# crispitagorico/sigkernel

Hardware: AMD Instinct MI355X
Metric: Gram entries/sec (fp64) (higher is better)
Workload: dtype f64; 1 GPU; BASELINE configs[2]: batch 512x512, len 128, dim 8, LinearKernel, dyadic 1, fp64, compute_Gram sym=False; step=compute_Gram, batch_x=512, rows_per_gpu=512, batch_y=512, len_x=128, len_y=128, dim=8, static_kernel=linear, dyadic_order=1, parallelism=SigKernel(process_group): gram rows sharded over 1 GPU(s), 1 all-gather per Gram

## Files before the change

### include/sigkernel_amd.h

```cpp
#ifndef SIGKERNEL_AMD_H
#define SIGKERNEL_AMD_H

#include <stddef.h>
#include <stdint.h>

#ifdef __cplusplus
extern "C" {
#endif

typedef enum sk_status {
    SK_OK = 0,
    SK_ERR_BAD_ARG = 1,
    SK_ERR_UNSUPPORTED = 2,
    SK_ERR_LAUNCH = 3,
    SK_ERR_WORKSPACE = 4,
    SK_ERR_NO_DEVICE = 5
} sk_status;

#define SK_SCHEME_DEFAULT 0
#define SK_SCHEME_NAIVE 1

#define SK_FLAG_NONE 0
#define SK_FLAG_EXACT 1
#define SK_FLAG_SIMPLE 2
#define SK_FLAG_EDGES_GIVEN 8
#define SK_FLAG_FAST_ONLY 4

int sk_version(void);
const char *sk_build_info(void);

#define SK_ROUTE_NO_STREAM 1
#define SK_ROUTE_NO_SWAP 2
double sk_cost_query(int which);
const char *sk_cost_name(int which);
const char *sk_cost_note(int which);
#define SK_OP_FORWARD 0
#define SK_OP_ADJOINT 1
#define SK_OP_ADJOINT_SYM 2
#define SK_OP_PREFIX 3
#define SK_OP_TRUNCATED 4
#define SK_OP_TRUNCATED_ADJOINT 5
#define SK_OP_TRUNCATED_RBF 6
#define SK_OP_TRUNCATED_RBF_ADJOINT 7
#define SK_OP_TRUNCATED_LONG 8
#define SK_OP_TRUNCATED_LONG_ADJOINT 9
#define SK_OP_TRUNCATED_WIDE_ADJOINT 10
#define SK_ROUTE_STREAM 0
#define SK_ROUTE_FUSED 1
#define SK_ROUTE_FUSED_MB 2
#define SK_ROUTE_FUSED_MB_SWAP 3
#define SK_ROUTE_FUSED_SWAP 4
int sk_route_query(int op, int kind, int D, int M, int N, int dyadic, int scheme, int elem_size, int flags);

void sk_reload_knobs(void);

int sk_launch_trace(int enable);
size_t sk_launch_trace_dump(char *buf, size_t n, int reset);

double sk_linear_prescale(int dyadic);
const char *sk_status_string(int status);
int sk_device_count(void);

int sk_increments_f64(const double *G, int64_t P, int M, int N, double *inc_c, int64_t ld, void *stream);
int sk_increments_f32(const float *G, int64_t P, int M, int N, float *inc_c, int64_t ld, void *stream);

int sk_static_increments_f64(int kind, double param, const double *X, const double *Y, int64_t A, int64_t B, int M, int N,
                             int D, double *inc_c, int64_t ld, void *stream);
int sk_static_increments_f32(int kind, double param, const float *X, const float *Y, int64_t A, int64_t B, int M, int N,
                             int D, float *inc_c, int64_t ld, void *stream);

int sk_static_adjoint_f64(int kind, double param, const double *X, const double *Y, const double *W, int64_t ldw,
                          const double *scale, int64_t A, int64_t B, int M, int N, int D, double *out, void *stream);
int sk_static_adjoint_f32(int kind, double param, const float *X, const float *Y, const float *W, int64_t ldw,
                          const float *scale, int64_t A, int64_t B, int M, int N, int D, float *out, void *stream);

int sk_linear_adjoint_f64(const double *dYt, int64_t ldy, const double *W, int64_t ldw, const double *scale, int64_t A,
                          int64_t B, int Mc, int Nc, int D, double *out, void *stream);
int sk_linear_adjoint_f32(const double *dYt, int64_t ldy, const float *W, int64_t ldw, const float *scale, int64_t A, int64_t B,
                          int Mc, int Nc, int D, float *out, void *stream);

int sk_linear_adjoint_fused_f64(const double *dXr, const double *dYt, int64_t A, int64_t B, int Mrows, int Mc, int Nc, int Ncp,
                                int dyadic, int scheme, const double *edges, const double *scale, double *tpart,
                                size_t tpart_doubles, double *err, double *ypart, size_t ypart_doubles, int *ppg_out, int *rows_out,
                                int *ycols_out, const double *kfinal, double screen, double tol, void *rescue_ws,
                                size_t rescue_ws_bytes, void *stream);

int sk_rbf_adjoint_fused_f64(const double *Xr, const double *Yt, int64_t A, int64_t B, int Mrows, int Mc, int Nc, int Ncp, int D,
                             int dyadic, int scheme, double sigma, const double *edges, const double *scale, double *gpart,
                             size_t gpart_doubles, double *err, double *ypart, size_t ypart_doubles, int *ppg_out, int *rows_out,
                             int *outw_out, int *ycols_out, const double *kfinal, double screen, double tol, void *rescue_ws,
                             size_t rescue_ws_bytes, void *stream);

size_t sk_solve_deriv_static_workspace_bytes(int64_t P, int Mc, int Nc, int dyadic, int D, int *mrows);
int sk_solve_deriv_static_f64(int kind, double param, const double *X0r, const double *X1r, const double *X2r, const double *Yt, int64_t A,
                              int64_t B, int Mrows, int Mc, int Nc, int Ncp, int D, int fd, int dyadic, int scheme, double eps, double *out_k,
                              double *out_kd, double *out_kdd, void *workspace, size_t workspace_bytes, void *stream);

int sk_rbf_adjoint_fused_mb_layout(int64_t P, int Mc, int Nc, int dyadic, int D, int *mrows, int *rows, int *outw, int *ncols,
                                   int64_t *edge_doubles, size_t *workspace_bytes);
int sk_rbf_adjoint_fused_mb_f64(const double *Xr, const void *Yt, int yt_f32, int64_t A, int64_t B, int Mrows, int Mc, int Nc, int Ncp, int D, int fd,
                                int dyadic, int scheme, double sigma, const double *edges, const double *scale, double *gpart,
                                size_t gpart_doubles, double *n0, size_t n0_doubles, double *err, void *workspace, size_t workspace_bytes,
                                const double *yt64, const double *kfinal, double screen, double tol, void *rescue_ws, size_t rescue_ws_bytes,
                                void *stream);

int sk_linear_adjoint_fused_mb_layout(int64_t P, int Mc, int Nc, int dyadic, int D, int *mrows, int *rows, int *outw, int64_t *edge_doubles,
                                      size_t *workspace_bytes);
int sk_linear_adjoint_fused_mb_f64(const double *dXr, const double *dYt, int64_t A, int64_t B, int Mrows, int Mc, int Nc, int Ncp, int D, int fd,
                                   int dyadic, int scheme, const double *edges, const double *scale, double *gpart, size_t gpart_doubles,
                                   double *err, void *workspace, size_t workspace_bytes, const double *kfinal, double screen, double tol,
                                   void *rescue_ws, size_t rescue_ws_bytes, void *stream);

// ... 199 lines not shown
```

### sigkernel_amd/_lib.py

```python
import ctypes
import os

import torch

from ._routes import routes

_HERE = os.path.dirname(os.path.abspath(__file__))
LIB_PATH = os.path.join(_HERE, "libsigkernel_amd.so")

SK_OK = 0
OP_FORWARD, OP_ADJOINT, OP_ADJOINT_SYM, OP_PREFIX, OP_TRUNCATED, OP_TRUNCATED_ADJOINT, OP_TRUNCATED_RBF = 0, 1, 2, 3, 4, 5, 6
OP_TRUNCATED_RBF_ADJOINT = 7
OP_TRUNCATED_LONG = 8
OP_TRUNCATED_LONG_ADJOINT = 9
OP_TRUNCATED_WIDE_ADJOINT = 10
ROUTE_STREAM, ROUTE_FUSED, ROUTE_FUSED_MB, ROUTE_FUSED_MB_SWAP, ROUTE_FUSED_SWAP = 0, 1, 2, 3, 4
ROUTE_NO_STREAM = 1
ROUTE_NO_SWAP = 2
SCHEME_DEFAULT = 0
SCHEME_NAIVE = 1
FLAG_EXACT = 1
FLAG_SIMPLE = 2
FLAG_FAST_ONLY = 4
FLAG_EDGES_GIVEN = 8
PREFIX_NODES = {"all": 0, "diagonal": 1, "last_row": 2, "last_col": 3}


def prefix_nodes_len(nodes, M, N):
    return {"diagonal": min(M, N), "last_row": N, "last_col": M}[nodes]

_lib = None

_vp = ctypes.c_void_p
_i64 = ctypes.c_int64
_int = ctypes.c_int
_sz = ctypes.c_size_t

SIGNATURES = {
    "sk_version": (_int, []),
    "sk_build_info": (ctypes.c_char_p, []),
    "sk_route_query": (_int, [_int, _int, _int, _int, _int, _int, _int, _int, _int]),
    "sk_cost_query": (ctypes.c_double, [_int]),
    "sk_cost_name": (ctypes.c_char_p, [_int]),
    "sk_cost_note": (ctypes.c_char_p, [_int]),
    "sk_solve_fwd_static_cols": (_int, [_int, _int]),
    "sk_reload_knobs": (None, []),
    "sk_launch_trace": (_int, [_int]),
    "sk_launch_trace_dump": (ctypes.c_size_t, [ctypes.c_char_p, ctypes.c_size_t, _int]),
    "sk_linear_prescale": (ctypes.c_double, [_int]),
    "sk_status_string": (ctypes.c_char_p, [_int]),
    "sk_device_count": (_int, []),
    "sk_increments_f64": (_int, [_vp, _i64, _int, _int, _vp, _i64, _vp]),
    "sk_increments_f32": (_int, [_vp, _i64, _int, _int, _vp, _i64, _vp]),
    "sk_static_increments_f64": (_int, [_int, ctypes.c_double, _vp, _vp, _i64, _i64, _int, _int, _int, _vp, _i64, _vp]),
    "sk_static_increments_f32": (_int, [_int, ctypes.c_double, _vp, _vp, _i64, _i64, _int, _int, _int, _vp, _i64, _vp]),
    "sk_static_adjoint_f64": (_int, [_int, ctypes.c_double, _vp, _vp, _vp, _i64, _vp, _i64, _i64, _int, _int, _int, _vp, _vp]),
    "sk_static_adjoint_f32": (_int, [_int, ctypes.c_double, _vp, _vp, _vp, _i64, _vp, _i64, _i64, _int, _int, _int, _vp, _vp]),
    "sk_linear_adjoint_f64": (_int, [_vp, _i64, _vp, _i64, _vp, _i64, _i64, _int, _int, _int, _vp, _vp]),
    "sk_linear_adjoint_f32": (_int, [_vp, _i64, _vp, _i64, _vp, _i64, _i64, _int, _int, _int, _vp, _vp]),
    "sk_static_adjoint2_f64": (_int, [_int, ctypes.c_double, _vp, _vp, _vp, _int, _vp, _i64, _vp, _i64, _i64, _int, _int, _int, _int,
                                      _vp, _vp]),
    "sk_static_adjoint2_f32": (_int, [_int, ctypes.c_double, _vp, _vp, _vp, _int, _vp, _i64, _vp, _i64, _i64, _int, _int, _int, _int,
                                      _vp, _vp]),
    "sk_increments_adjoint_f64": (_int, [_vp, _i64, _vp, _i64, _int, _int, _vp, _vp]),
    "sk_increments_adjoint_f32": (_int, [_vp, _i64, _vp, _i64, _int, _int, _vp, _vp]),
    "sk_solve_fwd_f64": (_int, [_vp, _i64, _i64, _int, _int, _int, _int, _int, _vp, _vp, _vp, _vp]),
    "sk_solve_fwd_f32": (_int, [_vp, _i64, _i64, _int, _int, _int, _int, _int, _vp, _vp, _vp, _vp]),
    "sk_solve_fwd_linear_f64": (_int, [_vp, _vp, _i64, _i64, _int, _int, _int, _int, _int, _int, _int, _vp, _vp, _vp]),
    "sk_solve_fwd_linear_f32": (_int, [_vp, _vp, _i64, _i64, _int, _int, _int, _int, _int, _int, _int, _vp, _vp, _vp]),
    "sk_solve_fwd_rbf_f64": (_int, [_vp, _vp, _i64, _i64, _int, _int, _int, _int, _int, _int, _int, ctypes.c_double, _vp, _vp, _vp]),
    "sk_solve_fwd_rbf_f32": (_int, [_vp, _vp, _i64, _i64, _int, _int, _int, _int, _int, _int, _int, ctypes.c_double, _vp, _vp, _vp]),
    "sk_solve_prefix_linear_f64": (_int, [_vp, _vp, _i64, _i64, _int, _int, _int, _int, _int, _int, _int, _vp, _i64, _vp, _vp]),
    "sk_solve_prefix_linear_f32": (_int, [_vp, _vp, _i64, _i64, _int, _int, _int, _int, _int, _int, _int, _vp, _i64, _vp, _vp]),
    "sk_solve_prefix_rbf_f64": (_int, [_vp, _vp, _i64, _i64, _int, _int, _int, _int, _int, _int, _int, ctypes.c_double, _vp, _i64, _vp, _vp]),
    "sk_solve_prefix_rbf_f32": (_int, [_vp, _vp, _i64, _i64, _int, _int, _int, _int, _int, _int, _int, ctypes.c_double, _vp, _i64, _vp, _vp]),
    "sk_solve_prefix_nodes_linear_f64": (_int, [_vp, _vp, _i64, _i64, _int, _int, _int, _int, _int, _int, _int, _int, _vp, _i64, _vp, _vp]),
    "sk_solve_prefix_nodes_linear_f32": (_int, [_vp, _vp, _i64, _i64, _int, _int, _int, _int, _int, _int, _int, _int, _vp, _i64, _vp, _vp]),
    "sk_solve_prefix_nodes_rbf_f64": (_int, [_vp, _vp, _i64, _i64, _int, _int, _int, _int, _int, _int, _int, ctypes.c_double, _int, _vp, _i64, _vp, _vp]),
    "sk_solve_prefix_nodes_rbf_f32": (_int, [_vp, _vp, _i64, _i64, _int, _int, _int, _int, _int, _int, _int, ctypes.c_double, _int, _vp, _i64, _vp, _vp]),
    "sk_solve_prefix_at_linear_f64": (_int, [_vp, _vp, _i64, _i64, _int, _int, _int, _int, _int, _int, _int, _vp, _vp, _vp, _vp, _vp]),
    "sk_solve_prefix_at_linear_f32": (_int, [_vp, _vp, _i64, _i64, _int, _int, _int, _int, _int, _int, _int, _vp, _vp, _vp, _vp, _vp]),
    "sk_solve_prefix_at_rbf_f64": (_int, [_vp, _vp, _i64, _i64, _int, _int, _int, _int, _int, _int, _int, ctypes.c_double, _vp, _vp, _vp, _vp, _vp]),
    "sk_solve_prefix_at_rbf_f32": (_int, [_vp, _vp, _i64, _i64, _int, _int, _int, _int, _int, _int, _int, ctypes.c_double, _vp, _vp, _vp, _vp, _vp]),
    "sk_truncated_gram_f64": (_int, [_vp, _vp, _i64, _i64, _int, _int, _int, _int, _int, _int, _int, _int, _vp, _vp, _vp]),
    "sk_truncated_gram_f32": (_int, [_vp, _vp, _i64, _i64, _int, _int, _int, _int, _int, _int, _int, _int, _vp, _vp, _vp]),
    "sk_truncated_paired_f64": (_int, [_vp, _vp, _i64, _int, _int, _int, _int, _int, _int, _int, _int, _vp, _vp, _vp]),
    "sk_truncated_paired_f32": (_int, [_vp, _vp, _i64, _int, _int, _int, _int, _int, _int, _int, _int, _vp, _vp, _vp]),
    "sk_truncated_levels_f64": (_int, [_vp, _vp, _i64, _i64, _int, _int, _int, _int, _int, _int, _int, _int, _vp, _vp]),
    "sk_truncated_levels_f32": (_int, [_vp, _vp, _i64, _i64, _int, _int, _int, _int, _int, _int, _int, _int, _vp, _vp]),
    "sk_truncated_levels_paired_f64": (_int, [_vp, _vp, _i64, _int, _int, _int, _int, _int, _int, _int, _int, _vp, _vp]),
    "sk_truncated_levels_paired_f32": (_int, [_vp, _vp, _i64, _int, _int, _int, _int, _int, _int, _int, _int, _vp, _vp]),
    "sk_truncated_points_f64": (_int, [_vp, _vp, _i64, _i64, _int, _int, _int, _int, _int, _int, _int, _int, _int, ctypes.c_double, _int, _int, _vp, _vp, _vp]),
    "sk_truncated_points_f32": (_int, [_vp, _vp, _i64, _i64, _int, _int, _int, _int, _int, _int, _int, _int, _int, ctypes.c_double, _int, _int, _vp, _vp, _vp]),
    "sk_truncated_long_plan": (_int, [_i64, _i64, _int, _int, _int, _int, _int, _sz, _vp]),
    "sk_truncated_long_f64": (_int, [_vp, _vp, _i64, _i64, _int, _int, _int, _int, _int, _int, _int, _int, _int, _int, _vp, _vp, _sz, _vp, _vp]),
    "sk_truncated_long_f32": (_int, [_vp, _vp, _i64, _i64, _int, _int, _int, _int, _int, _int, _int, _int, _int, _int, _vp, _vp, _sz, _vp, _vp]),
    "sk_truncated_adjoint_plan": (_int, [_i64, _i64, _int, _int, _int, _int, _int, _sz, _vp]),
    "sk_truncated_long_adjoint_plan": (_int, [_i64, _i64, _int, _int, _int, _int, _int, _sz, _vp]),
    "sk_truncated_long_adjoint": (_int, [_vp, _vp, _i64, _i64, _int, _int, _int, _int, _int, _int, _int, _vp, _vp, _i64, _vp, _sz, _vp, _int]),
    "sk_truncated_wide_adjoint_plan": (_int, [_i64, _i64, _int, _int, _int, _int, _int, _sz, _vp]),
    "sk_truncated_wide_adjoint": (_int, [_vp, _vp, _i64, _i64, _int, _int, _int, _int, _int, _int, _int, _vp, _vp, _i64, _vp, _sz, _vp, _int]),
    "sk_truncated_adjoint": (_int, [_vp, _vp, _i64, _i64, _int, _int, _int, _int, _int, _int, _int, _vp, _vp, _i64, _vp, _sz, _vp, _int]),
# ... 1447 lines not shown
```

### sigkernel_amd/csrc/sk_pair_stream.h

```cpp
#pragma once
#include "sk_wave_common.h"

namespace sk {
namespace {

__device__ __forceinline__ void lds_read_dims_issue(d2_t (&t)[8], unsigned a_even, unsigned a_odd) {
    asm volatile("ds_read_b128 %0, %8\n\t"
                 "ds_read_b128 %1, %9\n\t"
                 "ds_read_b128 %2, %8 offset:256\n\t"
                 "ds_read_b128 %3, %9 offset:256\n\t"
                 "ds_read_b128 %4, %8 offset:512\n\t"
                 "ds_read_b128 %5, %9 offset:512\n\t"
                 "ds_read_b128 %6, %8 offset:768\n\t"
                 "ds_read_b128 %7, %9 offset:768"
                 : "=&v"(t[0]), "=&v"(t[1]), "=&v"(t[2]), "=&v"(t[3]), "=&v"(t[4]), "=&v"(t[5]), "=&v"(t[6]), "=&v"(t[7])
                 : "v"(a_even), "v"(a_odd)
                 : "memory");
}
__device__ __forceinline__ void lds_read_dims_issue(d2_t (&t)[4], unsigned a_even, unsigned a_odd) {
    asm volatile("ds_read_b128 %0, %4\n\t"
                 "ds_read_b128 %1, %5\n\t"
                 "ds_read_b128 %2, %4 offset:256\n\t"
                 "ds_read_b128 %3, %5 offset:256"
                 : "=&v"(t[0]), "=&v"(t[1]), "=&v"(t[2]), "=&v"(t[3])
// ... 39 lines not shown
template <bool TRI, int FD, class PRM>
__device__ __forceinline__ int64_t pair_split(const PRM &prm, int64_t p, bool want_b) {
    if (prm.B <= 0) return p;
    if constexpr (TRI) {
        if (prm.tri) {
            const int *tab = reinterpret_cast<const int *>(prm.dYt + prm.B * (int64_t)FD * prm.Ncp);
            return (int64_t)tab[2 * p + (want_b ? 1 : 0)];
        }
    }
    if (want_b) return (int64_t)((uint32_t)p % (uint32_t)prm.B);
    return (int64_t)((uint32_t)p / (uint32_t)prm.B);
}


constexpr int x_window(int kind, int nd, int rc, bool edges) { return (kind == 0 && nd == 8 && rc == 4 && !edges) ? 4 : 8; }
constexpr int y_slab_pitch(int nd) { return nd * 128; }
constexpr int X_SLOTS = 2;
constexpr int x_row_bytes(int nd) { return nd == 4 ? 32 : 64; }

struct OneBandGeom {
    int NUp, logL, L, G, JMAX, GY;
    bool shy;
    size_t lds_bytes;
    int64_t n_pos;
};
struct OneBandShape {
    int kind, Mc, Nc, Mrows, Ncp, RC, nd;
    bool edges;
    int64_t A, B, P;
    int tri, logL_fixed;
};
inline int one_band_geometry(const OneBandShape &in, OneBandGeom &o) {
    const int NU = in.kind == 1 ? (in.Nc + 2) / 2 : (in.Nc + 1) / 2;
    const int rows = in.kind == 1 ? in.Mc + 1 : in.Mc;
    o.NUp = (NU + LINE_UNITS - 1) / LINE_UNITS * LINE_UNITS;
    if (in.Ncp < o.NUp * 2 || (in.Ncp & 1)) return SK_ERR_UNSUPPORTED;
    o.logL = 3;
    while (o.logL < 6 && (in.RC << o.logL) < rows) ++o.logL;
    if (in.logL_fixed > 0) o.logL = in.logL_fixed;
    o.L = 1 << o.logL;
    if (o.L * in.RC < rows) return SK_ERR_UNSUPPORTED;
    if (in.Mrows < o.L * in.RC) return SK_ERR_UNSUPPORTED;
    o.G = WAVE / o.L;
    o.JMAX = (o.L + o.NUp - 1) / o.NUp;
    o.shy = in.B > 0 && in.tri == 0 && !in.edges && o.G >= 2 && in.A > 0 && in.A <= 0x7fffffff && in.P == in.A * in.B;
    o.GY = o.shy ? 1 : o.G;
    o.lds_bytes = (size_t)o.GY * (((o.L >> 3) + 2) * y_slab_pitch(in.nd)) +
                  (size_t)o.G * (X_SLOTS * o.JMAX * in.RC * x_window(in.kind, in.nd, in.RC, in.edges) * x_row_bytes(in.nd));
    o.n_pos = o.shy ? (in.A + o.G - 1) / o.G * in.B : in.P;
    if (o.lds_bytes > 160 * 1024) return SK_ERR_UNSUPPORTED;
    return SK_OK;
}

inline void even_share(int64_t P, int G, int64_t max_waves, int64_t &waves, int64_t &per) {
    waves = (P + G - 1) / G;
    if (waves > max_waves) waves = max_waves;
    per = (P + waves * G - 1) / (waves * G);
}

struct StreamPlan {
    int64_t waves, per;
    int64_t q_first;
    int C0, n_big, logC;
    bool queue;
};
inline int plan_pair_stream(int64_t P, int G, int NUp, int L, int lag, int waves_per_cu, int n_cu, int pct, bool has_queue, StreamPlan &o) {
    const int64_t max_waves = (int64_t)n_cu * waves_per_cu;
    even_share(P, G, max_waves, o.waves, o.per);
    if (o.per > 0x1fffffff / NUp) return SK_ERR_UNSUPPORTED;
    if (P >= 0x7ff00000LL) return SK_ERR_UNSUPPORTED;
    const int span = (L - 1 + lag + 24) / NUp + 2;
    int logC = 0;
    while ((span >> logC) + 1 > 3) ++logC;
    while ((o.per * (100 - pct) / 100) >> (logC + 1) >= 24 && logC < 8) ++logC;
    o.logC = logC;
    o.queue = has_queue && o.waves == max_waves && o.per >= (8 << logC) && pct < 100;
    if (o.queue) {
        o.C0 = (int)(o.per * pct / 100);
        o.n_big = 0;
        o.q_first = o.waves * G * (int64_t)o.C0;
    } else {
        const int64_t base = P / (o.waves * G), rem = P - base * o.waves * G;
        o.C0 = (int)base;
        o.n_big = (int)((rem + G - 1) / G);
        if (base == 0) o.waves = o.n_big;
        o.q_first = P;
    }
    return SK_OK;
}

}
}
```

### sigkernel_amd/csrc/sk_wave_fused.hip

```cpp
#include "sk_pair_stream.h"
#include <algorithm>

namespace sk {
namespace {

constexpr int FD = 8;
struct FusedParams {
    const double *dXr;
    const double *dYt;
    void *out;
    double *edges;
    int64_t P, B;
    int Mrows, Ncp;
    int Mc, Nc, NUp, logL, PPG, n_steps;
    int u_f, lam_f, sel_f, naive;
    double inv_sigma;
    int dims;
    int e_NUp, e_L;
    int tri;
    WaveGroup wg;
    unsigned long long *queue;
    int64_t q_first;
    int C0, logC;
    int n_big;
    int rk_n, rk_wpr;
    unsigned long long rk_cnt;
    int shy_A;
};
template <int N>
__device__ __forceinline__ void lds_read_units(d2_t (&v)[N], unsigned addr);
__device__ __forceinline__ void lds_read_half_rows(d2_t (&v)[4], unsigned a) {
    asm volatile("ds_read_b128 %0, %4\n\t"
                 "ds_read_b128 %1, %4 offset:16\n\t"
                 "ds_read_b128 %2, %4 offset:64\n\t"
                 "ds_read_b128 %3, %4 offset:80\n\t"
                 "s_waitcnt lgkmcnt(0)"
                 : "=&v"(v[0]), "=&v"(v[1]), "=&v"(v[2]), "=&v"(v[3])
                 : "v"(a)
                 : "memory");
}
__device__ __forceinline__ void lds_read_line(d2_t (&v)[8], unsigned a) {
    asm volatile("ds_read_b128 %0, %8\n\t"
                 "ds_read_b128 %1, %8 offset:16\n\t"
                 "ds_read_b128 %2, %8 offset:32\n\t"
                 "ds_read_b128 %3, %8 offset:48\n\t"
                 "ds_read_b128 %4, %8 offset:64\n\t"
                 "ds_read_b128 %5, %8 offset:80\n\t"
                 "ds_read_b128 %6, %8 offset:96\n\t"
                 "ds_read_b128 %7, %8 offset:112\n\t"
                 "s_waitcnt lgkmcnt(0)"
                 : "=&v"(v[0]), "=&v"(v[1]), "=&v"(v[2]), "=&v"(v[3]), "=&v"(v[4]), "=&v"(v[5]), "=&v"(v[6]), "=&v"(v[7])
                 : "v"(a)
                 : "memory");
}
template <>
__device__ __forceinline__ void lds_read_units<4>(d2_t (&v)[4], unsigned a) {
    asm volatile("ds_read_b128 %0, %4\n\t"
                 "ds_read_b128 %1, %4 offset:16\n\t"
                 "ds_read_b128 %2, %4 offset:32\n\t"
                 "ds_read_b128 %3, %4 offset:48\n\t"
                 "s_waitcnt lgkmcnt(0)"
                 : "=&v"(v[0]), "=&v"(v[1]), "=&v"(v[2]), "=&v"(v[3])
                 : "v"(a)
                 : "memory");
}

template <typename TO, int DY, bool NAIVE, bool FULLWAVE, bool EDGES, int KIND, int ND, int RCX = 0>
__global__ __launch_bounds__(4 * WAVE) void k_fwd_fused(const FusedParams prm) {
    constexpr bool RBF = KIND == 1;
    constexpr bool AHEAD = !(RBF && EDGES && ND == 8);
    constexpr int LAG = RBF ? 2 : 0;
    constexpr int CW = 2;
    constexpr int RC = RCX ? RCX : Tile<DY>::RC, R = RC << DY, S = CW << DY, r = 1 << DY;
    constexpr int XROW = x_row_bytes(ND);
    constexpr int XW = x_window(KIND, ND, RC, EDGES);
    constexpr int XSLAB = RC * XW * XROW;
    constexpr int Y_SLAB_PITCH = y_slab_pitch(ND);
    extern __shared__ __attribute__((aligned(16))) char lds_block[];
    char *lds;
    const int64_t wave_id = wave_slot(prm.wg, lds_block, lds);
// ... 81 lines not shown
        int off;
        const int k = chunk_of(i, off);
        const int size = k == 0 ? C0 : CQ;
        left = size - 1 - off;
        const unsigned b = ring_at(k & 3);
        const unsigned p = b + (unsigned)((shy_a() > 0 ? 0 : g * size) + off);
        return (b >= P32 || p >= P32) ? NOPAIR : p;
    };
    auto stream_pair = [&](int g, int i) __attribute__((always_inline)) -> unsigned {
        int left;
        return stream_pair_left(g, i, left);
    };
    auto lane_pair = [&](int i) __attribute__((always_inline)) -> unsigned {
        int left;
        return stream_pair_left(grp, i, left);
    };
    auto ensure = [&](int f) __attribute__((always_inline)) {
        int off;
        const int kf = chunk_of(f, off);
        while (have <= kf) {
            unsigned b = NOPAIR;
            if (prm.queue && t_end == 0x7fffffff) {
                unsigned long long v = 0;
                if (lane == 0) v = atomicAdd(prm.queue, (unsigned long long)((shy_a() > 0 ? 1 : G) * CQ));
                const unsigned long long q = (unsigned long long)prm.q_first +
                                             (((unsigned long long)(unsigned)__builtin_amdgcn_readfirstlane((int)(v >> 32)) << 32) |
                                              (unsigned)__builtin_amdgcn_readfirstlane((int)v));
                b = q < (unsigned long long)P32 ? (unsigned)q : NOPAIR;
            }
            if (b == NOPAIR && t_end == 0x7fffffff)
                t_end = EDGES ? (C0 + (have - 1) * CQ) * NUp + (L - 1) + LAG
                              : (C0 + (have - 1) * CQ - 1) * NUp + prm.u_f + prm.lam_f + LAG + 1;
            const int kk = have & 3;
            const unsigned m0 = -(unsigned)(kk == 0), m1 = -(unsigned)(kk == 1), m2 = -(unsigned)(kk == 2), m3 = -(unsigned)(kk == 3);
            cb0 = (unsigned)__builtin_amdgcn_readfirstlane((int)((cb0 & ~m0) | (b & m0)));
            cb1 = (unsigned)__builtin_amdgcn_readfirstlane((int)((cb1 & ~m1) | (b & m1)));
            cb2 = (unsigned)__builtin_amdgcn_readfirstlane((int)((cb2 & ~m2) | (b & m2)));
            cb3 = (unsigned)__builtin_amdgcn_readfirstlane((int)((cb3 & ~m3) | (b & m3)));
            have += 1;
        }
    };
    const unsigned long long top_lanes = __builtin_amdgcn_ballot_w64(lam == 0);
    const unsigned my_y = lds0 + (shy ? 0u : (unsigned)grp * y_bytes);
    const unsigned y_lim = my_y + y_bytes;
    const unsigned ring_bytes = FULLWAVE ? (unsigned)(((WAVE >> 3) + 2) * Y_SLAB_PITCH) : y_bytes;
    {
        const unsigned ya = my_y + (unsigned)(yslab * Y_SLAB_PITCH + ((-lam & 7) << 4));
        a_e = ya + (unsigned)(ypar << 7);
    }
    const int JMAX = (L + NUp - 1) / NUp;
    const unsigned my_x = lds0 + x_base0 + (unsigned)((grp * X_SLOTS * JMAX) * XSLAB + (lam / NUp) * XSLAB) +
                          (unsigned)((lam & (XW - 1)) * RC * XROW);

    auto split_ab = [&](int64_t p, bool want_b) __attribute__((always_inline)) -> int64_t { return pair_split<true, FD>(prm, p, want_b); };
    auto split_b = [&](int64_t p) -> int64_t { return split_ab(p, true); };
    auto split_a = [&](int64_t p) -> int64_t { return split_ab(p, false); };
    int y_pi = 0, y_u0 = 0, y_slot = 0, y_par = 0;
    auto issue_y = [&]() __attribute__((always_inline)) {
        ensure(y_pi);
        const int gy = shy_a() > 0 ? 1 : G;
        for (int g = 0; g < gy; ++g) {
            const unsigned sp = stream_pair(g, y_pi);
            const int64_t p = sp == NOPAIR ? 0 : (int64_t)sp;
            const int64_t b = split_b(p);
            const int krow = (lane >> 3) ^ ((y_par + g) & 1);
            const double *src = prm.dYt + ((b * FD + krow) * (int64_t)prm.Ncp + (int64_t)(y_u0 + (lane & 7)) * 2);
            if (ND == 8 || lane < 32)
                __builtin_amdgcn_global_load_lds(src, (lds_void *)(lds + g * y_bytes + y_slot * Y_SLAB_PITCH), 16, 0, 0);
        }
        y_slot = y_slot + 1 == NSLAB ? 0 : y_slot + 1;
        y_par ^= 1;
        y_u0 += 8;
        if (y_u0 == NUp) { y_u0 = 0; y_pi += 1; }
    };
    int x_q0 = 0, x_lam0 = 0, x_slot = 0;
    auto issue_x = [&]() __attribute__((always_inline)) {
        ensure(x_q0);
        for (int j = 0; j < JMAX; ++j) {
            const int lamj = x_lam0 + j * NUp, pi = x_q0 - j;
            if (lamj >= L) break;
            const int sA = shy_a();
            const int64_t gm = sA > 0 ? G : 1, gs = sA > 0 ? 1 : 0, a_lim = sA > 0 ? sA : 0x7fffffff;
            for (int g = 0; g < G; ++g) {
                const unsigned sp = stream_pair(g, pi);
                const int64_t p = sp == NOPAIR ? 0 : (int64_t)sp;
                int64_t a = split_a(p);
                if constexpr (!EDGES && !FULLWAVE) {
                    a = a * gm + gs * g;
                    if (a >= a_lim) a = 0;
                }
                const char *src = reinterpret_cast<const char *>(prm.dXr + (a * prm.Mrows + (int64_t)lamj * RC) * FD);
                char *dst = lds + x_base0 + ((g * X_SLOTS + x_slot) * JMAX + j) * XSLAB;
#pragma unroll
                for (int c = 0; c < (XSLAB + 1023) / 1024; ++c)
                    if (c * 1024 + lane * 16 < XSLAB) {
                        const int so = XROW == 64 ? c * 1024 + lane * 16 : (c * 32 + (lane >> 1)) * 64 + (lane & 1) * 16;
                        __builtin_amdgcn_global_load_lds(src + so, (lds_void *)(dst + c * 1024), 16, 0, 0);
                    }
            }
        }
        x_slot = x_slot + 1 == X_SLOTS ? 0 : x_slot + 1;
        x_lam0 += XW;
        if (x_lam0 == NUp) { x_lam0 = 0; x_q0 += 1; }
    };

    d2_t dxq[RC][ND / 2];
#pragma unroll
    for (int k = 0; k < RC; ++k)
#pragma unroll
        for (int j = 0; j < ND / 2; ++j) dxq[k][j] = d2_t{0.0, 0.0};
    auto load_x_rows = [&](unsigned xa) {
        if constexpr (RC % 2 == 0 && ND == 8) {
#pragma unroll
            for (int k = 0; k < RC; k += 2) lds_load_line(dxq[k], dxq[k + 1], xa + k * 64u);
        } else if constexpr (RC % 2 == 0) {
#pragma unroll
            for (int k = 0; k < RC; k += 2) lds_load_two_half_rows(dxq[k], dxq[k + 1], xa + k * (unsigned)XROW);
        } else {
#pragma unroll
            for (int k = 0; k < RC; ++k) lds_load_row(dxq[k], xa + k * (unsigned)XROW);
        }
    };
    double own[RBF ? RC : 1][6], bel[4];
    constexpr bool PIN_EXP = RBF && !EDGES;
    ExpCoef expc;
    if (PIN_EXP) expc.init();
#pragma unroll
    for (int k = 0; k < (RBF ? RC : 1); ++k)
#pragma unroll
        for (int c = 0; c < 6; ++c) own[k][c] = 1.0;
#pragma unroll
    for (int c = 0; c < 4; ++c) bel[c] = 1.0;
    double left[R], bot[S], ktop[S], corner = 1.0;
#pragma unroll
    for (int i = 0; i < R; ++i) left[i] = 1.0;
#pragma unroll
    for (int i = 0; i < S; ++i) { bot[i] = 1.0; ktop[i] = 1.0; }

    const int EP = EDGES ? (prm.e_NUp * S + prm.e_L * R) : 0;
    int erow_lim = EDGES && lam == prm.lam_f ? prm.e_NUp : 0;
    int ecol_uf = EDGES && lam < prm.e_L ? prm.u_f : -1;
    int ecol_off = EDGES ? prm.e_NUp * S + lam * R : 0;
    asm volatile("" : "+v"(erow_lim), "+v"(ecol_uf), "+v"(ecol_off));
    double *ep_cur = nullptr, *nx_ptr = nullptr;
    int ep_left = 0, nx_left = 0;
    int ep_ok = 0, nx_ok = 0;
    int ep_k = 0;
    auto refresh_next = [&]() __attribute__((always_inline)) {
        if (EDGES) {
// ... 232 lines not shown
                    cbm[k][q] = fma(g2, -c_12, 1.0);
                }
            }

        double cand[RC][CW];
        double rowv[RC][S];
#pragma unroll
        for (int cc = 0; cc < S; ++cc) {
            double above = top[cc];
            double diag = cc == 0 ? corner : top[cc - 1];
#pragma unroll
            for (int rr = 0; rr < R; ++rr) {
                const double a = ca[rr >> DY][cc >> DY], b = cbm[rr >> DY][cc >> DY];
                const double k10 = left[rr];
                double v;
                if (NAIVE) v = fma(above, a, fma(k10, a, -diag));
                else v = fma(above, a, fma(k10, a, -(diag * b)));
                diag = k10;
                above = v;
                left[rr] = v;
                if ((rr & (r - 1)) == r - 1 && (cc & (r - 1)) == r - 1) cand[rr >> DY][cc >> DY] = v;
                if (EDGES && (rr & (r - 1)) == r - 1) rowv[rr >> DY][cc] = v;
            }
            bot[cc] = above;
        }
        if constexpr (RESET_AT_END) {
            asm volatile("v_mov_b64 %0, %1" : "=v"(corner) : "v"(top[S - 1]));
            take_top();
        } else if (!FULLWAVE) {
            corner = top[S - 1];
        }

        if (EDGES) {
            const bool pair_ok = ep_cur != nullptr;
            e_ptr = ep_cur;
            erow_at = (pair_ok && uk < erow_lim) ? uk * S : -1;
            ecol_at = (pair_ok && uk == ecol_uf) ? ecol_off : -1;
            if (!row_in_bot) {
#pragma unroll
                for (int kk = 0; kk < RC - 1; ++kk)
                    if (kk == k_f) {
#pragma unroll
                        for (int cc = 0; cc < S; ++cc) erow[cc] = rowv[kk][cc];
                    }
            }
        }

        if (__builtin_expect(CUR ? uk == my_uf : tm == c_out, 0)) {
            int pv = CUR ? psk : tq + c_kq + (tm + c_kr >= NUp ? 1 : 0);
            asm volatile("" : "+v"(pv));
            unsigned pair_u = lane_pair(pv);
            const int sA = shy_a();
            if (sA > 0 && pair_u != NOPAIR) {
                const unsigned Bu = (unsigned)prm.B, qa = pair_u / Bu, a = qa * (unsigned)G + (unsigned)grp;
                pair_u = a < (unsigned)sA ? a * Bu + (pair_u - qa * Bu) : NOPAIR;
            }
            const int64_t pair_v = (int64_t)pair_u;
            if (pair_u != NOPAIR) {
                double v = cand[0][0];
#pragma unroll
                for (int k = 0; k < RC; ++k)
#pragma unroll
                    for (int q = 0; q < CW; ++q) {
                        double cv = cand[k][q];
                        asm volatile("" : "+v"(cv));
                        if (k * CW + q == prm.sel_f) v = cv;
                    }
                if ((prm.tri & 3) == 1) {
                    const int *tab = reinterpret_cast<const int *>(prm.dYt + prm.B * (int64_t)FD * prm.Ncp);
                    const int64_t a = tab[2 * pair_v], b = tab[2 * pair_v + 1];
                    static_cast<TO *>(prm.out)[a * prm.B + b] = (TO)v;
                    static_cast<TO *>(prm.out)[b * prm.B + a] = (TO)v;
                } else {
                    static_cast<TO *>(prm.out)[pair_v] = (TO)v;
                }
            }
        }

        if constexpr (!CUR) {
            if constexpr (!MID && !RESET_AT_END) fetch_next();
            tm += 1;
            if (tm == NUp) { tm = 0; tq += 1; }
            if constexpr (RESET_AT_END) {
                asm volatile("" : "+s"(tq));
                fetch_next();
            }
        }
        if (CUR && RBF) {
            uk += 1;
            if (uk == NUp) {
                uk = 0;
                psk += 1;
                sweep_pair_is(psk);
            }
        }
        if constexpr (CUR) u += 1;
        if (CUR && ((t + 1) & 7) == lam7) {
            yslab = yslab + 1 == NSLAB ? 0 : yslab + 1;
            ypar ^= 1;
            if (u == NUp) {
                u = 0;
                ps += 1;
                if (!RBF) sweep_pair_is(ps);
            }
        }
        if (CUR && !RBF) { uk = u; psk = ps; }
        if (__builtin_expect(((t + 1) & (XW - 1)) == 0, 0)) {
// ... 170 lines not shown
    if (rbf0_two_rows && strip_edges && (g.naive || sizeof(TO) != 8)) return SK_ERR_UNSUPPORTED;
    const int nd_v = fused_nd(D, !g.naive && sizeof(TO) == 8);
    const int rcx = fused_rcx(KIND, DY, nd_v, strip_edges != nullptr, !g.naive && sizeof(TO) == 8);
    const int RC = rcx ? rcx : (DY == 0 ? 4 : DY == 1 ? 2 : 1);
    const bool doubled = rcx == 2 * (DY == 0 ? 4 : DY == 1 ? 2 : 1);
    int logL_fixed = 0;
    if (rbf0_two_rows && strip_edges) {
        const Strip st = strip_geom(rbf_edge_geom(g), 8);
        if (!st.ok || st.nb != 1 || st.logL > 5) return SK_ERR_UNSUPPORTED;
        logL_fixed = st.logL + 1;
    }
    const int nd = nd_v;
    OneBandGeom og;
    OneBandShape sh{};
    sh.kind = KIND, sh.Mc = g.Mc, sh.Nc = g.Nc, sh.Mrows = Mrows, sh.Ncp = Ncp, sh.RC = RC, sh.nd = nd;
    sh.edges = strip_edges != nullptr, sh.A = A, sh.B = B, sh.P = g.P, sh.tri = tri, sh.logL_fixed = logL_fixed;
    if (const int rc = one_band_geometry(sh, og)) return rc;
    const int NUp = og.NUp, logL = og.logL, L = og.L;
    const bool shy = og.shy;
    const size_t lds_bytes = og.lds_bytes;
    const int64_t n_pos = og.n_pos;

    int waves_per_cu = (int)((160 * 1024) / lds_bytes);
    const int wpc_env = knobs().fused_wpc;
    const int cap = wpc_env > 0 ? 16 : (DY == 0 ? 8 : (DY == 2 && nd == 4) ? 16 : 12);
    if (waves_per_cu > cap) waves_per_cu = cap;
    if (wpc_env > 0) waves_per_cu = waves_per_cu < wpc_env ? waves_per_cu : wpc_env;
    else if (waves_per_cu > 4) waves_per_cu &= ~3;
    if (waves_per_cu < 1) waves_per_cu = 1;
    const FusedPlan pl{n_pos, og.GY, NUp, L, KIND == 1 ? 2 : 0, lds_bytes, waves_per_cu, rcx};

    FusedParams prm;
    prm.dXr = dXr; prm.dYt = dYt; prm.out = out; prm.edges = strip_edges; prm.P = n_pos; prm.B = B;
    prm.Mrows = Mrows; prm.Ncp = Ncp; prm.Mc = g.Mc; prm.Nc = g.Nc; prm.NUp = NUp; prm.logL = logL;
    prm.inv_sigma = inv_sigma;
    prm.dims = D;
    prm.rk_n = 0; prm.rk_wpr = 1; prm.rk_cnt = 0;
    prm.tri = tri == 2 ? (2 | ((int)A << 2) | ((int)loss[0] << 17)) : tri;
    prm.queue = (unsigned long long *)queue;
    prm.e_NUp = NUp;
    prm.e_L = L;
    if (strip_edges) {
        const Strip st = strip_geom(KIND == 1 ? rbf_edge_geom(g) : g, 8);
        if (!st.ok || st.nb != 1 || (st.RC != RC && !rbf0_two_rows && !doubled) || ((1 << st.logL) * st.RC) % RC) return SK_ERR_UNSUPPORTED;
        prm.e_NUp = st.NUp;
        prm.e_L = ((1 << st.logL) * st.RC) / RC;
        if (prm.e_L > L) return SK_ERR_UNSUPPORTED;
    }
    prm.u_f = (g.Nc - 1) / 2;
    prm.lam_f = ((g.Mc - 1) / RC) % L;
    prm.sel_f = ((g.Mc - 1) % RC) * 2 + (g.Nc - 1) % 2;
    prm.naive = g.naive;
    prm.shy_A = shy ? (int)A : 0;
    switch (DY) {
        case 0: return launch_fused_dy<TO, 0, KIND>(prm, pl, s);
        case 1: return launch_fused_dy<TO, 1, KIND>(prm, pl, s);
        default: return launch_fused_dy<TO, 2, KIND>(prm, pl, s);
    }
}

}

template <typename TO>
int launch_fwd_fused_linear(const double *dXr, const double *dYt, int64_t A, int64_t B, int Mrows, int Ncp, int D, const Geom &g,
                            TO *out, double *strip_edges, void *queue, hipStream_t s, int tri, const int64_t *loss) {
    return launch_fwd_fused<TO, 0>(dXr, dYt, A, B, Mrows, Ncp, D, g, 0.0, out, strip_edges, queue, s, tri, loss);
}
template <typename TO>
int launch_fwd_fused_rbf(const double *Xr, const double *Yt, int64_t A, int64_t B, int Mrows, int Ncp, int D, const Geom &g,
                         double inv_sigma, TO *out, double *strip_edges, void *queue, hipStream_t s, int tri, const int64_t *loss) {
    return launch_fwd_fused<TO, 1>(Xr, Yt, A, B, Mrows, Ncp, D, g, inv_sigma, out, strip_edges, queue, s, tri, loss);
}

template int launch_fwd_fused_linear<double>(const double *, const double *, int64_t, int64_t, int, int, int, const Geom &, double *,
                                             double *, void *, hipStream_t, int, const int64_t *);
template int launch_fwd_fused_linear<float>(const double *, const double *, int64_t, int64_t, int, int, int, const Geom &, float *,
                                            double *, void *, hipStream_t, int, const int64_t *);
template int launch_fwd_fused_rbf<double>(const double *, const double *, int64_t, int64_t, int, int, int, const Geom &, double, double *,
                                          double *, void *, hipStream_t, int, const int64_t *);
template int launch_fwd_fused_rbf<float>(const double *, const double *, int64_t, int64_t, int, int, int, const Geom &, double, float *,
                                         double *, void *, hipStream_t, int, const int64_t *);

}
```

Baseline: 71.74 million entries/s.

## Use magic-number pair division and lane-broadcast pair indices in fused DMA issue

```diff
diff --git a/include/sigkernel_amd.h b/include/sigkernel_amd.h
--- a/include/sigkernel_amd.h
+++ b/include/sigkernel_amd.h
@@ -58,6 +58,7 @@
 size_t sk_launch_trace_dump(char *buf, size_t n, int reset);
 
 double sk_linear_prescale(int dyadic);
+int sk_pair_div_magic(int64_t B, uint32_t *mul, int *shift);
 const char *sk_status_string(int status);
 int sk_device_count(void);
 
diff --git a/sigkernel_amd/_lib.py b/sigkernel_amd/_lib.py
--- a/sigkernel_amd/_lib.py
+++ b/sigkernel_amd/_lib.py
@@ -48,6 +48,7 @@
     "sk_launch_trace": (_int, [_int]),
     "sk_launch_trace_dump": (ctypes.c_size_t, [ctypes.c_char_p, ctypes.c_size_t, _int]),
     "sk_linear_prescale": (ctypes.c_double, [_int]),
+    "sk_pair_div_magic": (_int, [_i64, ctypes.POINTER(ctypes.c_uint32), ctypes.POINTER(ctypes.c_int)]),
     "sk_status_string": (ctypes.c_char_p, [_int]),
     "sk_device_count": (_int, []),
     "sk_increments_f64": (_int, [_vp, _i64, _int, _int, _vp, _i64, _vp]),
diff --git a/sigkernel_amd/csrc/sk_pair_stream.h b/sigkernel_amd/csrc/sk_pair_stream.h
--- a/sigkernel_amd/csrc/sk_pair_stream.h
+++ b/sigkernel_amd/csrc/sk_pair_stream.h
@@ -115,6 +115,18 @@
     return SK_OK;
 }
 
+inline int div_magic(uint32_t B, unsigned &m, int &shift) {
+    if (B < 1 || B >= 0x80000000u) return 1;
+    int l = 0;
+    while ((1ull << l) < B) ++l;
+    const unsigned long long num = 1ull << (31 + l);
+    const unsigned long long mm = (num + B - 1) / B;
+    if (mm >> 32) return 1;
+    m = (unsigned)mm;
+    shift = l;
+    return 0;
+}
+
 inline void even_share(int64_t P, int G, int64_t max_waves, int64_t &waves, int64_t &per) {
     waves = (P + G - 1) / G;
     if (waves > max_waves) waves = max_waves;
diff --git a/sigkernel_amd/csrc/sk_wave_fused.hip b/sigkernel_amd/csrc/sk_wave_fused.hip
--- a/sigkernel_amd/csrc/sk_wave_fused.hip
+++ b/sigkernel_amd/csrc/sk_wave_fused.hip
@@ -26,6 +26,8 @@
     int rk_n, rk_wpr;
     unsigned long long rk_cnt;
     int shy_A;
+    unsigned div_m;
+    int div_s;
 };
 template <int N>
 __device__ __forceinline__ void lds_read_units(d2_t (&v)[N], unsigned addr);
@@ -213,21 +215,49 @@
     const unsigned my_x = lds0 + x_base0 + (unsigned)((grp * X_SLOTS * JMAX) * XSLAB + (lam / NUp) * XSLAB) +
                           (unsigned)((lam & (XW - 1)) * RC * XROW);
 
-    auto split_ab = [&](int64_t p, bool want_b) __attribute__((always_inline)) -> int64_t { return pair_split<true, FD>(prm, p, want_b); };
-    auto split_b = [&](int64_t p) -> int64_t { return split_ab(p, true); };
-    auto split_a = [&](int64_t p) -> int64_t { return split_ab(p, false); };
+    auto div_b = [&](unsigned p) __attribute__((always_inline)) -> unsigned {
+        unsigned m = prm.div_m;
+        int sh = prm.div_s;
+        asm volatile("" : "+s"(m), "+s"(sh));
+        return __umulhi(p << 1, m) >> sh;
+    };
+    auto split_ab = [&](unsigned p, bool want_b) __attribute__((always_inline)) -> int {
+        if (prm.B <= 0) return (int)p;
+        if (prm.tri) {
+            const int *tab = reinterpret_cast<const int *>(prm.dYt + prm.B * (int64_t)FD * prm.Ncp);
+            return __builtin_amdgcn_readfirstlane(tab[2 * (int64_t)p + (want_b ? 1 : 0)]);
+        }
+        const unsigned q = div_b(p);
+        return (int)(want_b ? p - q * (unsigned)prm.B : q);
+    };
+    constexpr bool PARK = !(EDGES && ((KIND == 0 && DY == 0 && ND == 4 && !FULLWAVE) || (KIND == 1 && DY == 2 && ND == 8 && FULLWAVE)));
+    int pos_ab = 0;
+    auto dma_lane = [&]() __attribute__((always_inline)) -> int {
+        int l = lane;
+        if constexpr (!PARK) asm volatile("" : "+v"(l));
+        return l;
+    };
+    const int NS = L >> 3;
     int y_pi = 0, y_u0 = 0, y_slot = 0, y_par = 0;
     auto issue_y = [&]() __attribute__((always_inline)) {
-        ensure(y_pi);
         const int gy = shy_a() > 0 ? 1 : G;
+        if constexpr (!PARK) pos_ab = 0;
+        const int ln = dma_lane();
+        if (!PARK || y_u0 == 0) {
+            ensure(y_pi);
+            for (int g = 0; g < gy; ++g) {
+                const unsigned sp = stream_pair(g, y_pi);
+                const int b = split_ab(sp == NOPAIR ? 0u : sp, true);
+                pos_ab = lane == 8 + g ? b : pos_ab;
+            }
+        }
         for (int g = 0; g < gy; ++g) {
-            const unsigned sp = stream_pair(g, y_pi);
-            const int64_t p = sp == NOPAIR ? 0 : (int64_t)sp;
-            const int64_t b = split_b(p);
-            const int krow = (lane >> 3) ^ ((y_par + g) & 1);
-            const double *src = prm.dYt + ((b * FD + krow) * (int64_t)prm.Ncp + (int64_t)(y_u0 + (lane & 7)) * 2);
-            if (ND == 8 || lane < 32)
-                __builtin_amdgcn_global_load_lds(src, (lds_void *)(lds + g * y_bytes + y_slot * Y_SLAB_PITCH), 16, 0, 0);
+            const int b = __builtin_amdgcn_readlane(pos_ab, 8 + g);
+            const int krow = (ln >> 3) ^ ((y_par + g) & 1);
+            const char *src = reinterpret_cast<const char *>(prm.dYt) + (int64_t)b * (FD * 8) * (int64_t)prm.Ncp;
+            const unsigned so = ((unsigned)krow * (unsigned)prm.Ncp + (unsigned)(y_u0 + (ln & 7)) * 2u) * 8u;
+            if (ND == 8 || ln < 32)
+                __builtin_amdgcn_global_load_lds(src + so, (lds_void *)(lds + g * y_bytes + y_slot * Y_SLAB_PITCH), 16, 0, 0);
         }
         y_slot = y_slot + 1 == NSLAB ? 0 : y_slot + 1;
         y_par ^= 1;
@@ -236,26 +266,42 @@
     };
     int x_q0 = 0, x_lam0 = 0, x_slot = 0;
     auto issue_x = [&]() __attribute__((always_inline)) {
-        ensure(x_q0);
+        if constexpr (!PARK) pos_ab = 0;
+        const int ln = dma_lane();
+        if (!PARK || x_lam0 == 0) {
+            ensure(x_q0);
+            const int sA = shy_a();
+            for (int jd = 0; jd < (PARK ? 1 : JMAX); ++jd) {
+                const int at = ((x_q0 - jd) & (NS - 1)) * G;
+                int qa = 0;
+                for (int g = 0; g < G; ++g) {
+                    if (sA <= 0 || g == 0) {
+                        const unsigned sp = stream_pair(g, x_q0 - jd);
+                        qa = split_ab(sp == NOPAIR ? 0u : sp, false);
+                    }
+                    int a = qa;
+                    if constexpr (!EDGES && !FULLWAVE) {
+                        if (sA > 0) {
+                            const int64_t ag = (int64_t)qa * G + g;
+                            a = ag >= sA ? 0 : (int)ag;
+                        }
+                    }
+                    pos_ab = lane == at + g ? a : pos_ab;
+                }
+            }
+        }
         for (int j = 0; j < JMAX; ++j) {
-            const int lamj = x_lam0 + j * NUp, pi = x_q0 - j;
+            const int lamj = x_lam0 + j * NUp;
             if (lamj >= L) break;
-            const int sA = shy_a();
-            const int64_t gm = sA > 0 ? G : 1, gs = sA > 0 ? 1 : 0, a_lim = sA > 0 ? sA : 0x7fffffff;
+            const int at = ((x_q0 - j) & (NS - 1)) * G;
             for (int g = 0; g < G; ++g) {
-                const unsigned sp = stream_pair(g, pi);
-                const int64_t p = sp == NOPAIR ? 0 : (int64_t)sp;
-                int64_t a = split_a(p);
-                if constexpr (!EDGES && !FULLWAVE) {
-                    a = a * gm + gs * g;
-                    if (a >= a_lim) a = 0;
-                }
-                const char *src = reinterpret_cast<const char *>(prm.dXr + (a * prm.Mrows + (int64_t)lamj * RC) * FD);
+                const int a = __builtin_amdgcn_readlane(pos_ab, at + g);
+                const char *src = reinterpret_cast<const char *>(prm.dXr + ((int64_t)a * prm.Mrows + (int64_t)lamj * RC) * FD);
                 char *dst = lds + x_base0 + ((g * X_SLOTS + x_slot) * JMAX + j) * XSLAB;
 #pragma unroll
                 for (int c = 0; c < (XSLAB + 1023) / 1024; ++c)
-                    if (c * 1024 + lane * 16 < XSLAB) {
-                        const int so = XROW == 64 ? c * 1024 + lane * 16 : (c * 32 + (lane >> 1)) * 64 + (lane & 1) * 16;
+                    if (c * 1024 + ln * 16 < XSLAB) {
+                        const unsigned so = XROW == 64 ? c * 1024 + ln * 16 : (c * 32 + (ln >> 1)) * 64 + (ln & 1) * 16;
                         __builtin_amdgcn_global_load_lds(src + so, (lds_void *)(dst + c * 1024), 16, 0, 0);
                     }
             }
@@ -594,7 +640,10 @@
             unsigned pair_u = lane_pair(pv);
             const int sA = shy_a();
             if (sA > 0 && pair_u != NOPAIR) {
-                const unsigned Bu = (unsigned)prm.B, qa = pair_u / Bu, a = qa * (unsigned)G + (unsigned)grp;
+                unsigned dm = prm.div_m;
+                int ds = prm.div_s;
+                asm volatile("" : "+s"(dm), "+s"(ds));
+                const unsigned Bu = (unsigned)prm.B, qa = __umulhi(pair_u << 1, dm) >> ds, a = qa * (unsigned)G + (unsigned)grp;
                 pair_u = a < (unsigned)sA ? a * Bu + (pair_u - qa * Bu) : NOPAIR;
             }
             const int64_t pair_v = (int64_t)pair_u;
@@ -871,6 +920,11 @@
     prm.sel_f = ((g.Mc - 1) % RC) * 2 + (g.Nc - 1) % 2;
     prm.naive = g.naive;
     prm.shy_A = shy ? (int)A : 0;
+    prm.div_m = 0; prm.div_s = 0;
+    if (B > 0) {
+        if (B >= 0x7ff00000LL || div_magic((uint32_t)B, prm.div_m, prm.div_s)) return SK_ERR_UNSUPPORTED;
+    }
+    if ((int64_t)Ncp * 64 >= 0x100000000LL) return SK_ERR_UNSUPPORTED;
     switch (DY) {
         case 0: return launch_fused_dy<TO, 0, KIND>(prm, pl, s);
         case 1: return launch_fused_dy<TO, 1, KIND>(prm, pl, s);
@@ -878,6 +932,16 @@
     }
 }
 
+}
+
+extern "C" int sk_pair_div_magic(int64_t B, uint32_t *mul, int *shift) {
+    if (!mul || !shift || B < 1 || B >= 0x80000000LL) return SK_ERR_BAD_ARG;
+    unsigned m = 0;
+    int sh = 0;
+    if (div_magic((uint32_t)B, m, sh)) return SK_ERR_BAD_ARG;
+    *mul = m;
+    *shift = sh;
+    return SK_OK;
 }
 
 template <typename TO>
```

After: 72.94 million entries/s, median of 6. +1.7%, better.
